# UVA-Computer-Vision-Lab/FrameINO

Hardware: AMD Instinct MI355X
Metric: denoise-steps/sec (Wan2.2-5B FrameINO, 49f 704x1280, cond+uncond DiT forward + CFG + Euler) (higher is better)
Workload: dtype bf16; 1 GPU; wan2.2-5b-49f-704x1280; layers=30, id_frames=1, hip_graph=False, parallelism=single, dead_rows_last_block=1760

## Files before the change

### frameino_amd/csrc/fino_attention_probs.hip

```cpp
#include <stdlib.h>

#include "fino_attention_common.h"
using namespace fino_attn_ns;

namespace {

struct ProbsParams {
    const uint16_t* q;
    const uint16_t* k;
    uint16_t* p;
    int batch, heads, lq, lk;
    int64_t q_bs, q_rs, q_hs, k_bs, k_rs, k_hs, p_bs, p_rs;
    int kp;
    const float* q_rrms;
    const uint16_t* q_weight;
    int64_t q_rrms_bs;
    float scale_log2;
    int lk_b[4];
    float log2_mult[4];
};

template <typename T, int NKB>
__global__ __launch_bounds__(256) void attn_probs_kernel(const ProbsParams p) {
    typedef typename T::vec8 vec8;
    __shared__ __attribute__((aligned(16))) char smem[4 * 8192];
    const int tid = threadIdx.x;
    const int lane = tid & 63;
    const int wave = tid >> 6;
    const int r = lane & 31;
    const int h = lane >> 5;
    const int hb = blockIdx.y;
    const int bi = hb / p.heads;
    const int head = hb - bi * p.heads;

    const int lkc = p.lk_b[bi < 4 ? bi : 3];
    const float lm = p.log2_mult[bi < 4 ? bi : 3];
    const int nkb = (lkc + 31) >> 5;
    const uint16_t* kp_ = p.k + bi * p.k_bs + head * p.k_hs;
    for (int i = 0; i < nkb * 2; ++i) {
        const int c = tid + 256 * i;
        const int row = c >> 4, ch = c & 15;
        uint4 u = make_uint4(0, 0, 0, 0);
        if (row < p.lk) u = *reinterpret_cast<const uint4*>(kp_ + (int64_t)row * p.k_rs + ch * 8);
        *reinterpret_cast<uint4*>(smem + row * 256 + ((ch ^ (row & 15)) << 4)) = u;
    }
    const int qrow = blockIdx.x * 128 + wave * 32 + r;
    const int qrc = qrow < p.lq ? qrow : p.lq - 1;
    const uint16_t* qp = p.q + bi * p.q_bs + head * p.q_hs + (int64_t)qrc * p.q_rs + 8 * h;
    vec8 qf[8];
    if (p.q_rrms) {
        const float rs = p.q_rrms[bi * p.q_rrms_bs + qrc];
        const uint16_t* wp = p.q_weight + head * 128 + 8 * h;
#pragma unroll
        for (int ks = 0; ks < 8; ++ks) {
            float f[8], ww[8];
            unpack8<T>(*reinterpret_cast<const uint4*>(qp + 16 * ks), f);
            unpack8<T>(*reinterpret_cast<const uint4*>(wp + 16 * ks), ww);
#pragma unroll
            for (int j = 0; j < 8; ++j) f[j] = round_to<T>(round_to<T>(f[j] * rs) * ww[j]);
            qf[ks] = __builtin_bit_cast(vec8, pack8<T>(f));
        }
    } else {
#pragma unroll
        for (int ks = 0; ks < 8; ++ks) qf[ks] = __builtin_bit_cast(vec8, *reinterpret_cast<const uint4*>(qp + 16 * ks));
    }
    __syncthreads();

    f32x16_t acc[NKB];
#pragma unroll
    for (int kb = 0; kb < NKB; ++kb)
#pragma unroll
        for (int j = 0; j < 16; ++j) acc[kb][j] = 0.f;
#pragma unroll
    for (int kb = 0; kb < NKB; ++kb) {
        if (kb < nkb) {
#pragma unroll
            for (int ks = 0; ks < 8; ++ks) {
                const int row = kb * 32 + r;
                const uint4 a = *reinterpret_cast<const uint4*>(smem + row * 256 + (((2 * ks + h) ^ (row & 15)) << 4));
                acc[kb] = T::mfma32(__builtin_bit_cast(vec8, a), qf[ks], acc[kb]);
            }
        }
    }

    const float c2 = p.scale_log2;
    float m = -INFINITY;
#pragma unroll
    for (int kb = 0; kb < NKB; ++kb) {
#pragma unroll
        for (int j = 0; j < 16; ++j) {
            const int key = kb * 32 + (j & 3) + 8 * (j >> 2) + 4 * h;
            float x = acc[kb][j] * c2;
            x = key == lkc - 1 ? x + lm : x;
            x = key >= lkc ? -INFINITY : x;
            acc[kb][j] = x;
            m = fmaxf(m, x);
        }
    }
    {
        const auto sw = __builtin_amdgcn_permlane32_swap(__float_as_uint(m), __float_as_uint(m), false, false);
        m = fmaxf(__uint_as_float(sw[0]), __uint_as_float(sw[1]));
    }
    float l = 0.f;
#pragma unroll
    for (int kb = 0; kb < NKB; ++kb) {
#pragma unroll
        for (int j = 0; j < 16; ++j) {
            const float e = __builtin_amdgcn_exp2f(acc[kb][j] - m);
            acc[kb][j] = e;
            l += e;
        }
    }
    {
        const auto sw = __builtin_amdgcn_permlane32_swap(__float_as_uint(l), __float_as_uint(l), false, false);
        l = __uint_as_float(sw[0]) + __uint_as_float(sw[1]);
    }
    const float inv = 1.0f / l;
    __syncthreads();
    char* stage = smem + wave * 8192;
#pragma unroll
    for (int kb = 0; kb < NKB; ++kb) {
#pragma unroll
        for (int g4 = 0; g4 < 4; ++g4) {
            const int key0 = kb * 32 + 8 * g4 + 4 * h;
            if (key0 < p.kp) {
                const uint32_t w0 = (uint32_t)T::from_f32(acc[kb][4 * g4 + 0] * inv) | ((uint32_t)T::from_f32(acc[kb][4 * g4 + 1] * inv) << 16);
                const uint32_t w1 = (uint32_t)T::from_f32(acc[kb][4 * g4 + 2] * inv) | ((uint32_t)T::from_f32(acc[kb][4 * g4 + 3] * inv) << 16);
                *reinterpret_cast<uint2*>(stage + r * 256 + ((((key0 >> 3)) ^ (r & 15)) << 4) + ((key0 & 4) << 1)) = make_uint2(w0, w1);
            }
        }
    }
    __syncthreads();
    const int pieces = p.kp >> 3;
    const int total = 32 * pieces;
    const int row_base = blockIdx.x * 128 + wave * 32;
    uint16_t* pbase = p.p + bi * p.p_bs + head * p.kp;
    for (int i = lane; i < total; i += 64) {
        const int rr = i / pieces, pc = i - rr * pieces;
        const uint4 u = *reinterpret_cast<const uint4*>(stage + rr * 256 + ((pc ^ (rr & 15)) << 4));
        if (row_base + rr < p.lq) *reinterpret_cast<uint4*>(pbase + (int64_t)(row_base + rr) * p.p_rs + pc * 8) = u;
    }
}

}

extern "C" int fino_attn_probs_supported(int batch, int heads, int64_t lq, int64_t lk, int head_dim) {
    return head_dim == 128 && batch >= 1 && batch <= 4 && heads > 0 && lq > 0 && lk >= 1 && lk <= 128 &&
           (int64_t)batch * heads <= 65535;
}

extern "C" int fino_attn_probs(const void* q, const void* k, void* p, int batch, int heads, int64_t lq, int64_t lk,
                               int head_dim, int64_t q_bs, int64_t q_rs, int64_t q_hs, int64_t k_bs, int64_t k_rs, int64_t k_hs,
                               int kp, int64_t p_bs, int64_t p_rs, float scale, int dtype, const int* lk_b,
                               const float* tail_mult, const float* q_rrms, int64_t q_rrms_bs, const void* q_weight,
                               void* stream) {
    FINO_CHECK((q_rrms == nullptr) == (q_weight == nullptr) && fino_aligned16(q_weight), FINO_ERR_ARG,
               "fino_attn_probs: q_rrms and q_weight come together (q_weight 16-byte aligned)");
    FINO_CHECK(dtype == FINO_BF16 || dtype == FINO_F16, FINO_ERR_ARG, "fino_attn_probs: dtype %d", dtype);
    FINO_CHECK(q && k && p && lk_b && tail_mult, FINO_ERR_ARG, "fino_attn_probs: null pointer");
    FINO_CHECK(fino_attn_probs_supported(batch, heads, lq, lk, head_dim), FINO_ERR_UNSUPPORTED,
               "fino_attn_probs: needs head_dim 128, batch <= 4, lk <= 128 (got head_dim %d, batch %d, lk %lld)", head_dim, batch,
               (long long)lk);
    FINO_CHECK(fino_aligned16(q) && fino_aligned16(k) && fino_aligned16(p) && q_rs % 8 == 0 && k_rs % 8 == 0 && q_hs % 8 == 0 &&
                   k_hs % 8 == 0 && q_bs % 8 == 0 && k_bs % 8 == 0 && p_bs % 8 == 0 && p_rs % 8 == 0,
               FINO_ERR_ARG, "fino_attn_probs: pointers and strides must be 16-byte aligned");
    FINO_CHECK(kp > 0 && kp % 8 == 0 && kp <= 128 && p_rs >= (int64_t)heads * kp, FINO_ERR_ARG,
               "fino_attn_probs: kp %d (a multiple of 8, <= 128), row stride %lld", kp, (long long)p_rs);
    FINO_CHECK(scale > 0.f || scale == FINO_ATTN_SCALE_FOLDED, FINO_ERR_ARG, "fino_attn_probs: scale");
    if (lq == 0) return FINO_OK;
    ProbsParams pp;
    pp.q = (const uint16_t*)q; pp.k = (const uint16_t*)k; pp.p = (uint16_t*)p;
    pp.batch = batch; pp.heads = heads; pp.lq = (int)lq; pp.lk = (int)lk;
    pp.q_bs = q_bs; pp.q_rs = q_rs; pp.q_hs = q_hs; pp.k_bs = k_bs; pp.k_rs = k_rs; pp.k_hs = k_hs; pp.p_bs = p_bs; pp.p_rs = p_rs;
    pp.kp = kp;
    pp.q_rrms = q_rrms; pp.q_weight = (const uint16_t*)q_weight; pp.q_rrms_bs = q_rrms_bs;
    pp.scale_log2 = scale == FINO_ATTN_SCALE_FOLDED ? 1.0f : scale * 1.4426950408889634f;
    for (int b = 0; b < 4; ++b) {
        const int bb = b < batch ? b : batch - 1;
        FINO_CHECK(lk_b[bb] >= 1 && lk_b[bb] <= lk && lk_b[bb] <= kp && tail_mult[bb] >= 1.0f, FINO_ERR_ARG,
                   "fino_attn_probs: lk_b[%d] = %d (of %lld, kp %d), tail_mult %g", bb, lk_b[bb], (long long)lk, kp,
                   (double)tail_mult[bb]);
        pp.lk_b[b] = lk_b[bb];
        pp.log2_mult[b] = log2f(tail_mult[bb]);
    }
    hipStream_t st = (hipStream_t)stream;
    const dim3 grid((unsigned)((lq + 127) / 128), (unsigned)(batch * heads));
    int max_lk = 0;
    for (int b = 0; b < batch; ++b) max_lk = lk_b[b] > max_lk ? lk_b[b] : max_lk;
    const int need = max_lk > kp ? max_lk : kp;
    const int nkb = need <= 64 ? 2 : (need <= 96 ? 3 : 4);
#define PROBS_LAUNCH(T_)                                                                                      \
    {                                                                                                         \
        if (nkb == 2) attn_probs_kernel<T_, 2><<<grid, 256, 0, st>>>(pp);                                     \
        else if (nkb == 3) attn_probs_kernel<T_, 3><<<grid, 256, 0, st>>>(pp);                                \
        else attn_probs_kernel<T_, 4><<<grid, 256, 0, st>>>(pp);                                              \
    }
    if (dtype == FINO_BF16) PROBS_LAUNCH(BF16) else PROBS_LAUNCH(F16)
#undef PROBS_LAUNCH
    FINO_LAUNCH_CHECK();
    return FINO_OK;
}
```

Measured before the change: 3.739 denoise-steps/s.

## Make attention-probs kernel persistent over query blocks, reusing staged K in LDS

The probs kernel now launches a grid sized to fill CUs by LDS occupancy, and each workgroup loops over a contiguous range of 128-row query blocks. K is loaded into LDS once per workgroup and reused across those blocks, and the next block's Q rows are prefetched into registers during the current block's compute. Fully valid key blocks skip the masking logic, the output staging uses a separate LDS region with wave-level fences instead of block barriers, and a reciprocal multiply replaces the integer division. The trade-offs are a larger LDS footprint, which limits occupancy, and a risk of load imbalance across workgroups; this kernel is probably a small share of the DiT step.

After: 3.740 denoise-steps/s (median of 5 runs). Within noise of the previous version (+0.0%).

```diff
diff --git a/frameino_amd/csrc/fino_attention_probs.hip b/frameino_amd/csrc/fino_attention_probs.hip
--- a/frameino_amd/csrc/fino_attention_probs.hip
+++ b/frameino_amd/csrc/fino_attention_probs.hip
@@ -20,10 +20,20 @@
     float log2_mult[4];
 };
 
+constexpr int probs_lds_bytes(int nkb) { return (nkb + 4) * 8192 + 256; }
+
+inline int probs_grid_x(int64_t nblk, int bh, int cus, int per_cu) {
+    int64_t n = (int64_t)cus * per_cu / bh;
+    n = n < 1 ? 1 : n;
+    return (int)(n < nblk ? n : nblk);
+}
+
+constexpr int probs_per_cu(int nkb) { return 160 * 1024 / probs_lds_bytes(nkb); }
+
 template <typename T, int NKB>
-__global__ __launch_bounds__(256) void attn_probs_kernel(const ProbsParams p) {
+__global__ __launch_bounds__(256, probs_per_cu(NKB)) void attn_probs_kernel(const ProbsParams p) {
     typedef typename T::vec8 vec8;
-    __shared__ __attribute__((aligned(16))) char smem[4 * 8192];
+    __shared__ __attribute__((aligned(16))) char smem[probs_lds_bytes(NKB)];
     const int tid = threadIdx.x;
     const int lane = tid & 63;
     const int wave = tid >> 6;
@@ -33,9 +43,16 @@
     const int bi = hb / p.heads;
     const int head = hb - bi * p.heads;
 
-    const int lkc = p.lk_b[bi < 4 ? bi : 3];
+    const int nblk = (p.lq + 127) >> 7;
+    const int per = nblk / (int)gridDim.x, rem = nblk - per * (int)gridDim.x;
+    const int g = blockIdx.x;
+    int blk = g * per + (g < rem ? g : rem);
+    const int blk_end = blk + per + (g < rem ? 1 : 0);
+    if (blk >= blk_end) return;
+
+    const int lkc_wg = p.lk_b[bi < 4 ? bi : 3];
     const float lm = p.log2_mult[bi < 4 ? bi : 3];
-    const int nkb = (lkc + 31) >> 5;
+    const int nkb = (lkc_wg + 31) >> 5;
     const uint16_t* kp_ = p.k + bi * p.k_bs + head * p.k_hs;
     for (int i = 0; i < nkb * 2; ++i) {
         const int c = tid + 256 * i;
@@ -44,102 +61,154 @@
         if (row < p.lk) u = *reinterpret_cast<const uint4*>(kp_ + (int64_t)row * p.k_rs + ch * 8);
         *reinterpret_cast<uint4*>(smem + row * 256 + ((ch ^ (row & 15)) << 4)) = u;
     }
-    const int qrow = blockIdx.x * 128 + wave * 32 + r;
-    const int qrc = qrow < p.lq ? qrow : p.lq - 1;
-    const uint16_t* qp = p.q + bi * p.q_bs + head * p.q_hs + (int64_t)qrc * p.q_rs + 8 * h;
-    vec8 qf[8];
-    if (p.q_rrms) {
-        const float rs = p.q_rrms[bi * p.q_rrms_bs + qrc];
-        const uint16_t* wp = p.q_weight + head * 128 + 8 * h;
-#pragma unroll
-        for (int ks = 0; ks < 8; ++ks) {
-            float f[8], ww[8];
-            unpack8<T>(*reinterpret_cast<const uint4*>(qp + 16 * ks), f);
-            unpack8<T>(*reinterpret_cast<const uint4*>(wp + 16 * ks), ww);
-#pragma unroll
-            for (int j = 0; j < 8; ++j) f[j] = round_to<T>(round_to<T>(f[j] * rs) * ww[j]);
-            qf[ks] = __builtin_bit_cast(vec8, pack8<T>(f));
-        }
-    } else {
-#pragma unroll
-        for (int ks = 0; ks < 8; ++ks) qf[ks] = __builtin_bit_cast(vec8, *reinterpret_cast<const uint4*>(qp + 16 * ks));
+    const uint16_t* qbase = p.q + bi * p.q_bs + head * p.q_hs + 8 * h;
+    const float* rrp = p.q_rrms ? p.q_rrms + bi * p.q_rrms_bs : nullptr;
+    char* wsm = smem + (NKB + 4) * 8192;
+    if (rrp && tid < 16) *reinterpret_cast<uint4*>(wsm + tid * 16) = *reinterpret_cast<const uint4*>(p.q_weight + head * 128 + tid * 8);
+    uint4 qn[8];
+    float rsn = 0.f;
+    {
+        const int qrow = blk * 128 + wave * 32 + r;
+        const int qrc = qrow < p.lq ? qrow : p.lq - 1;
+        const uint16_t* qp = qbase + (int64_t)qrc * p.q_rs;
+#pragma unroll
+        for (int ks = 0; ks < 8; ++ks) qn[ks] = *reinterpret_cast<const uint4*>(qp + 16 * ks);
+        if (rrp) rsn = rrp[qrc];
     }
     __syncthreads();
 
-    f32x16_t acc[NKB];
-#pragma unroll
-    for (int kb = 0; kb < NKB; ++kb)
-#pragma unroll
-        for (int j = 0; j < 16; ++j) acc[kb][j] = 0.f;
-#pragma unroll
-    for (int kb = 0; kb < NKB; ++kb) {
-        if (kb < nkb) {
-#pragma unroll
-            for (int ks = 0; ks < 8; ++ks) {
-                const int row = kb * 32 + r;
-                const uint4 a = *reinterpret_cast<const uint4*>(smem + row * 256 + (((2 * ks + h) ^ (row & 15)) << 4));
-                acc[kb] = T::mfma32(__builtin_bit_cast(vec8, a), qf[ks], acc[kb]);
-            }
-        }
-    }
-
-    const float c2 = p.scale_log2;
-    float m = -INFINITY;
-#pragma unroll
-    for (int kb = 0; kb < NKB; ++kb) {
-#pragma unroll
-        for (int j = 0; j < 16; ++j) {
-            const int key = kb * 32 + (j & 3) + 8 * (j >> 2) + 4 * h;
-            float x = acc[kb][j] * c2;
-            x = key == lkc - 1 ? x + lm : x;
-            x = key >= lkc ? -INFINITY : x;
-            acc[kb][j] = x;
-            m = fmaxf(m, x);
-        }
-    }
-    {
-        const auto sw = __builtin_amdgcn_permlane32_swap(__float_as_uint(m), __float_as_uint(m), false, false);
-        m = fmaxf(__uint_as_float(sw[0]), __uint_as_float(sw[1]));
-    }
-    float l = 0.f;
-#pragma unroll
-    for (int kb = 0; kb < NKB; ++kb) {
-#pragma unroll
-        for (int j = 0; j < 16; ++j) {
-            const float e = __builtin_amdgcn_exp2f(acc[kb][j] - m);
-            acc[kb][j] = e;
-            l += e;
-        }
-    }
-    {
-        const auto sw = __builtin_amdgcn_permlane32_swap(__float_as_uint(l), __float_as_uint(l), false, false);
-        l = __uint_as_float(sw[0]) + __uint_as_float(sw[1]);
-    }
-    const float inv = 1.0f / l;
-    __syncthreads();
-    char* stage = smem + wave * 8192;
-#pragma unroll
-    for (int kb = 0; kb < NKB; ++kb) {
-#pragma unroll
-        for (int g4 = 0; g4 < 4; ++g4) {
-            const int key0 = kb * 32 + 8 * g4 + 4 * h;
-            if (key0 < p.kp) {
-                const uint32_t w0 = (uint32_t)T::from_f32(acc[kb][4 * g4 + 0] * inv) | ((uint32_t)T::from_f32(acc[kb][4 * g4 + 1] * inv) << 16);
-                const uint32_t w1 = (uint32_t)T::from_f32(acc[kb][4 * g4 + 2] * inv) | ((uint32_t)T::from_f32(acc[kb][4 * g4 + 3] * inv) << 16);
-                *reinterpret_cast<uint2*>(stage + r * 256 + ((((key0 >> 3)) ^ (r & 15)) << 4) + ((key0 & 4) << 1)) = make_uint2(w0, w1);
-            }
-        }
-    }
-    __syncthreads();
+    char* stage = smem + NKB * 8192 + wave * 8192;
     const int pieces = p.kp >> 3;
     const int total = 32 * pieces;
-    const int row_base = blockIdx.x * 128 + wave * 32;
+    const uint32_t pieces_rcp = (65536u + pieces - 1) / pieces;
     uint16_t* pbase = p.p + bi * p.p_bs + head * p.kp;
-    for (int i = lane; i < total; i += 64) {
-        const int rr = i / pieces, pc = i - rr * pieces;
-        const uint4 u = *reinterpret_cast<const uint4*>(stage + rr * 256 + ((pc ^ (rr & 15)) << 4));
-        if (row_base + rr < p.lq) *reinterpret_cast<uint4*>(pbase + (int64_t)(row_base + rr) * p.p_rs + pc * 8) = u;
-    }
+    const float c2 = p.scale_log2;
+
+    for (; blk < blk_end; ++blk) {
+        vec8 qf[8];
+        if (rrp) {
+            const float rs = rsn;
+#pragma unroll
+            for (int ks = 0; ks < 8; ++ks) {
+                float f[8], ww[8];
+                unpack8<T>(qn[ks], f);
+                unpack8<T>(*reinterpret_cast<const uint4*>(wsm + (16 * ks + 8 * h) * 2), ww);
+#pragma unroll
+                for (int j = 0; j < 8; ++j) f[j] = round_to<T>(round_to<T>(f[j] * rs) * ww[j]);
+                qf[ks] = __builtin_bit_cast(vec8, pack8<T>(f));
+            }
+        } else {
+#pragma unroll
+            for (int ks = 0; ks < 8; ++ks) qf[ks] = __builtin_bit_cast(vec8, qn[ks]);
+        }
+        if (blk + 1 < blk_end) {
+            const int qrow = (blk + 1) * 128 + wave * 32 + r;
+            const int qrc = qrow < p.lq ? qrow : p.lq - 1;
+            const uint16_t* qp = qbase + (int64_t)qrc * p.q_rs;
+#pragma unroll
+            for (int ks = 0; ks < 8; ++ks) qn[ks] = *reinterpret_cast<const uint4*>(qp + 16 * ks);
+            if (rrp) rsn = rrp[qrc];
+        }
+
+        f32x16_t acc[NKB];
+#pragma unroll
+        for (int kb = 0; kb < NKB; ++kb)
+#pragma unroll
+            for (int j = 0; j < 16; ++j) acc[kb][j] = 0.f;
+#pragma unroll
+        for (int kb = 0; kb < NKB; ++kb) {
+            if (kb < nkb) {
+#pragma unroll
+                for (int ks = 0; ks < 8; ++ks) {
+                    const int row = kb * 32 + r;
+                    const uint4 a = *reinterpret_cast<const uint4*>(smem + row * 256 + (((2 * ks + h) ^ (row & 15)) << 4));
+                    acc[kb] = T::mfma32(__builtin_bit_cast(vec8, a), qf[ks], acc[kb]);
+                }
+            }
+        }
+
+        int lkc = lkc_wg;
+        asm volatile("" : "+s"(lkc));
+        float m = -INFINITY;
+#pragma unroll
+        for (int kb = 0; kb < NKB; ++kb) {
+            if (kb * 32 + 32 < lkc) {
+#pragma unroll
+                for (int j = 0; j < 16; ++j) {
+                    const float x = acc[kb][j] * c2;
+                    acc[kb][j] = x;
+                    m = fmaxf(m, x);
+                }
+            } else if (kb * 32 < lkc) {
+#pragma unroll
+                for (int j = 0; j < 16; ++j) {
+                    const int key = kb * 32 + (j & 3) + 8 * (j >> 2) + 4 * h;
+                    float x = acc[kb][j] * c2;
+                    x = key == lkc - 1 ? x + lm : x;
+                    x = key >= lkc ? -INFINITY : x;
+                    acc[kb][j] = x;
+                    m = fmaxf(m, x);
+                }
+            }
+        }
+        {
+            const auto sw = __builtin_amdgcn_permlane32_swap(__float_as_uint(m), __float_as_uint(m), false, false);
+            m = fmaxf(__uint_as_float(sw[0]), __uint_as_float(sw[1]));
+        }
+        float l = 0.f;
+#pragma unroll
+        for (int kb = 0; kb < NKB; ++kb) {
+            if (kb * 32 < lkc) {
+#pragma unroll
+                for (int j = 0; j < 16; ++j) {
+                    const float e = __builtin_amdgcn_exp2f(acc[kb][j] - m);
+                    acc[kb][j] = e;
+                    l += e;
+                }
+            }
+        }
+        {
+            const auto sw = __builtin_amdgcn_permlane32_swap(__float_as_uint(l), __float_as_uint(l), false, false);
+            l = __uint_as_float(sw[0]) + __uint_as_float(sw[1]);
+        }
+        const float inv = 1.0f / l;
+        __builtin_amdgcn_fence(__ATOMIC_ACQ_REL, "wavefront");
+#pragma unroll
+        for (int kb = 0; kb < NKB; ++kb) {
+#pragma unroll
+            for (int g4 = 0; g4 < 4; ++g4) {
+                const int key0 = kb * 32 + 8 * g4 + 4 * h;
+                if (key0 < p.kp) {
+                    const uint32_t w0 = (uint32_t)T::from_f32(acc[kb][4 * g4 + 0] * inv) | ((uint32_t)T::from_f32(acc[kb][4 * g4 + 1] * inv) << 16);
+                    const uint32_t w1 = (uint32_t)T::from_f32(acc[kb][4 * g4 + 2] * inv) | ((uint32_t)T::from_f32(acc[kb][4 * g4 + 3] * inv) << 16);
+                    *reinterpret_cast<uint2*>(stage + r * 256 + ((((key0 >> 3)) ^ (r & 15)) << 4) + ((key0 & 4) << 1)) = make_uint2(w0, w1);
+                }
+            }
+        }
+        __builtin_amdgcn_fence(__ATOMIC_ACQ_REL, "wavefront");
+        const int row_base = blk * 128 + wave * 32;
+        for (int i = lane; i < total; i += 64) {
+            const int rr = (int)(((uint32_t)i * pieces_rcp) >> 16), pc = i - rr * pieces;
+            const uint4 u = *reinterpret_cast<const uint4*>(stage + rr * 256 + ((pc ^ (rr & 15)) << 4));
+            if (row_base + rr < p.lq) *reinterpret_cast<uint4*>(pbase + (int64_t)(row_base + rr) * p.p_rs + pc * 8) = u;
+        }
+    }
+}
+
+struct ProbsDevice { int cus, lds_per_cu; };
+ProbsDevice probs_device() {
+    static std::atomic<int> cus[kFinoMaxDevices], lds[kFinoMaxDevices];
+    const int dev = fino_current_device();
+    ProbsDevice d = {cus[dev].load(std::memory_order_relaxed), lds[dev].load(std::memory_order_relaxed)};
+    if (d.cus == 0 || d.lds_per_cu == 0) {
+        hipDeviceProp_t prop;
+        const bool ok = hipGetDeviceProperties(&prop, dev) == hipSuccess;
+        d.cus = ok && prop.multiProcessorCount > 0 ? prop.multiProcessorCount : 256;
+        d.lds_per_cu = ok && prop.maxSharedMemoryPerMultiProcessor > 0 ? (int)prop.maxSharedMemoryPerMultiProcessor : 160 * 1024;
+        cus[dev].store(d.cus, std::memory_order_relaxed);
+        lds[dev].store(d.lds_per_cu, std::memory_order_relaxed);
+    }
+    return d;
 }
 
 }
@@ -184,11 +253,14 @@
         pp.log2_mult[b] = log2f(tail_mult[bb]);
     }
     hipStream_t st = (hipStream_t)stream;
-    const dim3 grid((unsigned)((lq + 127) / 128), (unsigned)(batch * heads));
     int max_lk = 0;
     for (int b = 0; b < batch; ++b) max_lk = lk_b[b] > max_lk ? lk_b[b] : max_lk;
     const int need = max_lk > kp ? max_lk : kp;
     const int nkb = need <= 64 ? 2 : (need <= 96 ? 3 : 4);
+    const ProbsDevice dv = probs_device();
+    int per_cu = dv.lds_per_cu / probs_lds_bytes(nkb);
+    per_cu = per_cu < 1 ? 1 : (per_cu > probs_per_cu(nkb) ? probs_per_cu(nkb) : per_cu);
+    const dim3 grid((unsigned)probs_grid_x((lq + 127) / 128, batch * heads, dv.cus, per_cu), (unsigned)(batch * heads));
 #define PROBS_LAUNCH(T_)                                                                                      \
     {                                                                                                         \
         if (nkb == 2) attn_probs_kernel<T_, 2><<<grid, 256, 0, st>>>(pp);                                     \
```
